# simplerr/rust-renderer

Measured on AMD Instinct MI355X. Metric: Mrays/s (path rays: primary + bounce + sun-shadow + light-shadow) at 1920x1080, 20 spp = 20 frames x 1 spp; camera and sun at rest, the one-off builds of the camera grid and the sun grid outside the timed region (value_with_grid_builds charges them to these frames, value_tree_walk uses neither grid), higher is better.
Workload: dtype f32

## Files before the change

### rust-renderer_amd/csrc/context_state.h

```cpp
#pragma once
#include <hip/hip_runtime.h>

#include <string>
#include <utility>
#include <vector>

#include "bvh.h"
#include "context_internal.h"
#include "device_types.h"
#include "grid_cache.h"
#include "utopian_hip.h"

using namespace uh;

struct HostMesh {
   std::vector<UhVertex> vertices;
   std::vector<uint32_t> indices;
   UhGpuMaterial material;
   float o2w[12];
   float w2o[9];
   bool iso = false, iso_reference = true;
   uint32_t iso_res = 0;
   float iso_lo = 0.0f, iso_hi = 0.0f;
   bool dev = false, host_valid = true;
// ... 297 lines not shown
   bool furnace = false;
   uint64_t frames = 0;
   float build_ms = 0.0f, last_frame_ms = 0.0f;
   float ms_by_kind[5] = {0, 0, 0, 0, 0};
   uint32_t trace_closest_launches = 0, trace_light_launches = 0;
   bool frame_timed = false;
   std::vector<EventPair> pending, free_events;
   uint32_t bvh_nodes = 0, bvh_tris = 0;

   bool sun_grid_enabled = true;
   uint64_t geom_version = 1;
   CachedGrid<3> sun;
   SunGridExtras sun_x;
   bool primary_implicit = true;
   bool slim_state = true;

   bool cam_grid_enabled = true;
   CachedGrid<32> cam;

   struct __attribute__((visibility("hidden"))) Tiles {
      uint32_t rank = 0, world = 1, tile = 64;
      DevBuf<uint32_t> owned_pixels;
      uint32_t n_owned = 0;
      DevBuf<float4> send, recv;
      hipEvent_t ev_compose = nullptr;
      void destroy() {
         owned_pixels.release(), send.release(), recv.release();
         if (ev_compose) (void)hipEventDestroy(ev_compose);
      }
   } tiles;
// ... 299 lines not shown
```

### rust-renderer_amd/csrc/device_types.h

```cpp
#pragma once
#include <hip/hip_runtime.h>

#include <cstdint>
#include <vector>

#include "bvh.h"
#include "frame_plan.h"
#include "path_layout.h"
#include "post_levels.h"
#include "sun_grid.h"
#include "utopian_hip.h"

namespace uh {

constexpr uint32_t kMaxBounces = 64;
constexpr uint32_t kQueueKinds = 5;
enum { Q_RAY = 0, Q_LIGHT = 1, Q_SUN_TREE = 2, Q_MISS = 3, Q_CAM_TREE = 4 };
constexpr uint32_t kLaunchSlots = kMaxBounces * 4 + 8;

constexpr uint32_t kShards = 32;
constexpr uint32_t kShardBits = 5;
static_assert((1u << kShardBits) == kShards, "kShards is a power of two");
static_assert(kLayoutShards == kShards && kLayoutShardBits == kShardBits, "path_layout.h states the same shards");
__host__ __device__ inline uint32_t shard_of_run(uint32_t run) { return (run * 0x9E3779B1u) >> (32 - kShardBits); }
// ... 331 lines not shown
struct LaunchCfg {
   hipStream_t stream;
   uint32_t num_cus;
   uint32_t closest_blocks_per_cu, shadow_blocks_per_cu;
   bool count_visits;
   uint32_t fused_blocks_per_cu = 4;
};

void launch_generate(const LaunchCfg&, const FrameParams&, const PathState&, Control*, uint32_t sample);
void launch_trace_closest(const LaunchCfg&, const SceneDev&, const PathState&, Control*, DeviceStats*, uint32_t bounce, uint32_t cursor_slot,
                          int ray_kind);
void launch_trace_camera_grid(const LaunchCfg&, const FrameParams&, const SceneDev&, const PathState&, Control*, DeviceStats*, uint32_t cursor_slot_grid, uint32_t cursor_slot_tree,
                              const SunGridDev&, bool leftovers_possible = true);
void launch_shade_miss(const LaunchCfg&, const FrameParams&, const PathState&, Control*, DeviceStats*, uint32_t bounce);
void launch_shade_hit(const LaunchCfg&, const FrameParams&, const SceneDev&, const PathState&, const Images&, Control*, DeviceStats*, uint32_t bounce);
void launch_flush_survivors(const LaunchCfg&, const FrameParams&, const PathState&, Control*);
void launch_path_fused(const LaunchCfg&, const FrameParams&, const SceneDev&, const PathState&, Control*, DeviceStats*, const SunGridDev& g, bool use_grid, bool sun_of_bounce0);
void launch_trace_shadow(const LaunchCfg&, const FrameParams&, const SceneDev&, const PathState&, Control*, DeviceStats*, uint32_t bounce,
                         uint32_t cursor_slot, bool light, bool sun_leftovers = false);
void launch_trace_sun_grid(const LaunchCfg&, const FrameParams&, const SceneDev&, const PathState&, Control*, DeviceStats*, uint32_t bounce,
                           uint32_t cursor_slot, const SunGridDev&);
void launch_finish_sample(const LaunchCfg&, const FrameParams&, const PathState&, const Images&, uint32_t sample, bool last);
void launch_resolve(const LaunchCfg&, const Images&, uint32_t W, uint32_t H, uint32_t total_samples, uint32_t limit);
void launch_gbuffer(const LaunchCfg&, const FrameParams&, const SceneDev&, const RawRays&, const Images&, DeviceStats*, const RowSpans& spans, uint32_t counted,
                    const SunGridDev* camera_grid = nullptr);
void launch_reset_reservoirs(const LaunchCfg&, const FrameParams&, const Images&, const RowSpans& spans);
void launch_initial_ris(const LaunchCfg&, const FrameParams&, const SceneDev&, const Images&, const RowSpans& spans);
void launch_temporal_reuse(const LaunchCfg&, const FrameParams&, const SceneDev&, const Images&, const RowSpans& spans);
void launch_spatial_reuse(const LaunchCfg&, const FrameParams&, const SceneDev&, const Images&, const RowSpans& spans);
void launch_trace_closest_raw(const LaunchCfg&, const SceneDev&, const float4* ray_o, const float4* ray_d, float4* hit, uint32_t n);
// ... 171 lines not shown
```

### rust-renderer_amd/csrc/frame_loop.hip

```cpp
#include <hip/hip_runtime.h>

#include <algorithm>
#include <cmath>
#include <cstring>
#include <string>

#include "context_internal.h"
#include "context_state.h"
#include "device_types.h"
#include "frame_plan.h"
#include "tile_partition.h"
#include "utopian_hip.h"

using namespace uh;

FrameParams make_params(uh_ctx* c, const UhViewUniformData& v) {
   FrameParams fp;
   std::memset(&fp, 0, sizeof(fp));
   std::memcpy(fp.inv_view, v.inverse_view, sizeof(fp.inv_view));
   std::memcpy(fp.inv_proj, v.inverse_projection, sizeof(fp.inv_proj));
   std::memcpy(fp.prev_pv, v.prev_frame_projection_view, sizeof(fp.prev_pv));
   float d = (v.sun_dir[0] * v.sun_dir[0] + v.sun_dir[1] * v.sun_dir[1]) + v.sun_dir[2] * v.sun_dir[2];
   float inv = 1.0f / std::sqrt(d);
   for (int a = 0; a < 3; a++) fp.sun_dir[a] = v.sun_dir[a] * inv;
// ... 46 lines not shown
      if (c->last_acc == s.ev_acc) c->last_acc = nullptr;
      for (hipEvent_t& r : c->spatial_reader)
         if (r == s.ev_acc) r = nullptr;
      if (c->t_start == s.frame_start) c->t_start = nullptr;
      if (c->t_stop == s.frame_stop) c->t_stop = nullptr;
      s.destroy();
   }
   HIP_TRY(c, s.create(need));
   return UH_OK;
}

static int enqueue_path_trace(uh_ctx* c, Slot& s, const FrameParams& frame) {
   FrameParams fp = frame;
   LaunchCfg lc = cfg(c);
   lc.stream = s.stream;
   const SampleOptions opt{c->fused_bounces, c->fused_always, c->sun_x.verdicts, c->slim_state, c->overlap_miss, c->overlap_shadow, lc.closest_blocks_per_cu, lc.shadow_blocks_per_cu};
   const SampleFacts facts{fp.batch_frames, fp.num_bounces, fp.samples_per_frame, fp.n_owned, s.ps.shard_cap, fp.sun_shadow_enabled == 1, fp.lights_enabled == 1,
                           c->sun.this_frame, c->cam.this_frame};
   Control* ctl = s.control.p;
   DeviceStats* st = c->dstats.p;
   for (uint32_t smp = 0; smp < fp.samples_per_frame; smp++) {
      uint32_t slot = 0;
      const bool gpu_idle = !c->last_acc || hipEventQuery(c->last_acc) == hipSuccess;
      const SamplePlan plan = plan_sample(opt, facts, gpu_idle);
      lc.closest_blocks_per_cu = plan.closest_blocks_per_cu;
      lc.shadow_blocks_per_cu = plan.shadow_blocks_per_cu;
      fp.sun_verdicts = plan.sun_verdicts ? 1u : 0u;
      fp.slim_state = plan.slim_state ? 1u : 0u;
      HIP_TRY(c, hipMemsetAsync(ctl, 0, sizeof(Control), s.stream));
      launch_generate(lc, fp, s.ps, ctl, smp);
      for (uint32_t b = 0; b < plan.wave_bounces; b++) {
         begin_timed(c, (b == 0 && plan.grid_primary) ? 3 : 0, s.stream);
         if (b == 0 && plan.grid_primary) {
            launch_trace_camera_grid(lc, fp, c->scene, s.ps, ctl, st, slot, slot + 1, c->cam.dev, c->cam.max_list_interior > std::max(c->cam.dev.walk_whole, c->cam.dev.max_walk));
            slot += 2;
         } else
            launch_trace_closest(lc, c->scene, s.ps, ctl, st, b, slot++, b == 0 ? UH_RAY_PRIMARY : UH_RAY_BOUNCE);
         end_timed(c, s.stream);
         if (plan.side_used && b > 0) HIP_TRY(c, hipStreamWaitEvent(s.stream, s.ev_shadowed, 0));
         begin_timed(c, 2, s.stream);
         launch_shade_hit(lc, fp, c->scene, s.ps, c->im, ctl, st, b);
         if (!c->overlap_miss) launch_shade_miss(lc, fp, s.ps, ctl, st, b);
         end_timed(c, s.stream);
         LaunchCfg lsh = lc;
         hipStream_t sh_stream = s.stream;
         if (plan.side_used) {
            HIP_TRY(c, hipEventRecord(s.ev_shaded, s.stream));
            HIP_TRY(c, hipStreamWaitEvent(s.side, s.ev_shaded, 0));
         }
         if (c->overlap_miss) {
            LaunchCfg ls = lc;
            ls.stream = s.side;
            begin_timed(c, 2, s.side);
            launch_shade_miss(ls, fp, s.ps, ctl, st, b);
            end_timed(c, s.side);
         }
// ... 281 lines not shown
```

### rust-renderer_amd/csrc/frame_plan.h

```cpp
#pragma once
#include <cstdint>

#include "utopian_hip.h"

namespace uh {

constexpr uint32_t kMaxBatchFrames = 32;
constexpr uint32_t kRestirBatch = 16;
constexpr uint32_t kFusedMaxPaths = 4u << 20;
constexpr uint32_t kSingleFrameBlocksPerCu = 4;

struct SampleOptions {
   bool fused_bounces, fused_always, sun_verdicts, slim_state, overlap_miss, overlap_shadow;
   uint32_t closest_blocks_per_cu, shadow_blocks_per_cu;
};
struct SampleFacts {
   uint32_t batch_frames, num_bounces, samples_per_frame, n_owned, shard_cap;
   bool sun_shadow_enabled, lights_enabled;
   bool sun_grid, camera_grid;
};
struct SamplePlan {
   bool fused;
   bool fused_sun0;
   bool sun_verdicts;
   bool slim_state;
   uint32_t closest_blocks_per_cu, shadow_blocks_per_cu;
   bool grid_primary;
   bool side_shadow;
   bool side_used;
   bool join_side;
   uint32_t wave_bounces;
   bool flush;
};

inline SamplePlan plan_sample(const SampleOptions& o, const SampleFacts& f, bool gpu_idle) {
   SamplePlan p;
   const bool lone = f.batch_frames == 1;
   p.closest_blocks_per_cu = lone && o.closest_blocks_per_cu > kSingleFrameBlocksPerCu ? kSingleFrameBlocksPerCu : o.closest_blocks_per_cu;
   p.shadow_blocks_per_cu = lone && o.shadow_blocks_per_cu > kSingleFrameBlocksPerCu ? kSingleFrameBlocksPerCu : o.shadow_blocks_per_cu;
   p.fused = o.fused_bounces && f.batch_frames == 1 && f.num_bounces >= 2 && f.num_bounces <= 64 && f.shard_cap < (1u << 23) &&
             ((gpu_idle && f.n_owned <= kFusedMaxPaths) || o.fused_always);
   p.fused_sun0 = p.fused && f.sun_shadow_enabled && !f.lights_enabled;
   p.sun_verdicts = o.sun_verdicts && f.sun_grid && f.sun_shadow_enabled && !f.lights_enabled && !p.fused;
   p.slim_state = o.slim_state && p.sun_verdicts && f.samples_per_frame == 1;
   p.grid_primary = f.camera_grid;
   p.side_shadow = o.overlap_shadow && (f.sun_shadow_enabled || f.lights_enabled);
   p.side_used = p.side_shadow || o.overlap_miss;
   p.join_side = (o.overlap_miss || o.overlap_shadow) && f.num_bounces > 0;
   p.wave_bounces = p.fused ? 1u : f.num_bounces;
   p.flush = f.num_bounces > 0 && !p.fused && !p.slim_state;
   return p;
}

inline uint32_t plan_batch_size(uint32_t option, uint64_t owned, uint32_t pass_mask) {
   uint32_t batch = option;
   if (!batch) {
      uint64_t b = (32u << 20) / (owned ? owned : 1), cap = (33u << 20) / (owned ? owned : 1);
      if (b > cap) b = cap;
      batch = (uint32_t)(b < 1 ? 1 : b);
   }
   if (batch > kMaxBatchFrames) batch = kMaxBatchFrames;
   if ((pass_mask & UH_PASS_RESTIR) && batch > kRestirBatch) batch = kRestirBatch;
   if (!(pass_mask & UH_PASS_REFERENCE_PT)) batch = 1;
   return batch;
}
// ... 8 lines not shown
```

### rust-renderer_amd/csrc/kernels.hip

```cpp
#include <hip/hip_runtime.h>

#include "device_math.h"
#include "device_types.h"
#include "grid_walk.h"
#include "kernel_common.h"
#include "path_shading.h"
#include "traversal.h"

namespace uh {

template <bool COUNT>
__global__ __launch_bounds__(kBlock, 6) void k_trace_closest(SceneDev sc, bool sharded, const float4* __restrict__ ray_o,
                                                               const float4* __restrict__ ray_d, float4* __restrict__ hit_out, uint32_t shard_cap, Control* ctl,
                                                               DeviceStats* stats, uint32_t bounce, uint32_t cursor_slot, int ray_kind, uint32_t raw_count,
                                                               const uint32_t* __restrict__ listed) {
   const bool range_in_w = !sharded;
   __shared__ uint32_t s_stack[kWavesPerBlock][kLdsStack][64];
   __shared__ RayPool<2> s_pool[kWavesPerBlock];
   const uint32_t lane = lane_id();
   const uint32_t wave = threadIdx.x >> 6;
   uint32_t* lds_col = &s_stack[wave][0][lane];
   RayPool<2>& pool = s_pool[wave];
   RaySource src;
   uint32_t seg = 0;
// ... 318 lines not shown
            if (defer[k]) st_stream(q_tree + slot, id[k]);
         }
      });
   }
   if (sx.lb == 0 && threadIdx.x == 0) {
      atomicAdd(&stats->rays[UH_RAY_SUN_SHADOW], (unsigned long long)count);
      if (COUNT) atomicAdd(&stats->shadow_nodes_visited, (unsigned long long)count);
   }
   if (COUNT) {
      atomicAdd(&stats->shadow_tris_tested, (unsigned long long)n_tris);
      atomicAdd(&stats->sun_covered_rays, (unsigned long long)n_covered);
   }
}

template <bool COUNT>
__global__ __launch_bounds__(kBlock) void k_trace_camera_grid(SceneDev sc, FrameParams fp, PathState ps, Control* ctl, DeviceStats* stats, uint32_t cursor_slot, SunGridDev g) {
   const uint32_t lane = lane_id();
   const ShardCtx sx = shard_ctx();
   const uint32_t seg = sx.shard * ps.shard_cap;
   const uint32_t* __restrict__ queue = ps.queue[0] + seg;
   const uint32_t count = ctl->q_count[qc_index(0, Q_RAY, sx.shard)];
   uint32_t* cursor = &ctl->cursor[cursor_index(cursor_slot, sx.shard)];
   const PathRecs rec = ps.set[0];
   const float4* __restrict__ tris = sc.tris;
   uint32_t* q_tree = ps.queue[3] + seg;
   uint32_t* n_tree = &ctl->q_count[qc_index(0, Q_CAM_TREE, sx.shard)];
   uint32_t n_tris = 0;
   for (;;) {
      const uint32_t base = next_batch(cursor);
      if (base >= count) break;
// ... 12 lines not shown
         defer = end - e > (g.walk_whole > g.max_walk ? g.walk_whole : g.max_walk);
         if (defer && fp.primary_implicit) {
            float4 ro, rd;
            primary_state(fp, id, ro, rd);
            st_rec(rec_quad(rec, seg + i, REC_ORIGIN), ro);
            st_rec(rec_quad(rec, seg + i, REC_DIR), rd);
         }
         if (!defer) {
            float4 ro, rd;
            if (fp.primary_implicit)
               primary_state(fp, id, ro, rd);
            else {
               ro = ld_rec(rec_quad(rec, seg + i, REC_ORIGIN));
               rd = ld_rec(rec_quad(rec, seg + i, REC_DIR));
            }
            const V3 o = v3(ro.x, ro.y, ro.z), d = v3(rd.x, rd.y, rd.z);
            Hit best;
            best.t = 10000.0f;
            best.u = best.v = 0.0f;
            best.idx = kEmptyRef;
            best.key = 0xffffffffu;
            uint2 en = make_uint2(0u, 0u);
            if (e < end) en = reinterpret_cast<const uint2*>(g.entries)[e];
            while (e < end) {
               if (sorted && -__uint_as_float(en.y) > best.t) break;
               const uint32_t pk = en.x;
               uint2 nxt = make_uint2(0u, 0u);
               if (e + 1 < end) nxt = reinterpret_cast<const uint2*>(g.entries)[e + 1];
               const float4 a = tris[kTriStride16 * (size_t)pk + 0], b = tris[kTriStride16 * (size_t)pk + 1], c = tris[kTriStride16 * (size_t)pk + 2];
               if (COUNT) n_tris++;
               tri_compute<false>(a, b, c, pk, o, d, 0.001f, INFINITY, best);
               en = nxt;
               e++;
            }
            st_rec(ps.hit + seg + i, make_float4(best.t, best.u, best.v, __uint_as_float(best.idx)));
         }
      }
      if (__ballot(defer) != 0ull) {
         const uint32_t slot = wave_append(n_tree, defer);
         if (defer) st_stream(q_tree + slot, i);
      }
   }
   if (sx.lb == 0 && threadIdx.x == 0) atomicAdd(&stats->rays[UH_RAY_PRIMARY], (unsigned long long)count);
   if (COUNT) atomicAdd(&stats->cam_tris_tested, (unsigned long long)n_tris);
}

__global__ __launch_bounds__(kBlock) void k_gbuffer_camera_grid(SceneDev sc, RawRays ps, RowSpans spans, uint32_t W, SunGridDev g) {
   const uint32_t n = spans.total();
   const float4* __restrict__ tris = sc.tris;
// ... 82 lines not shown
   const ShardCtx sx = shard_ctx();
   const uint32_t seg = sx.shard * ps.shard_cap;
   const uint2* __restrict__ queue = reinterpret_cast<const uint2*>(ps.queue[4]) + seg;
   const uint32_t count = ctl->q_count[qc_index(bounce, Q_MISS, sx.shard)];
   for (uint32_t i = sx.lb * kBlock + threadIdx.x; i < count; i += sx.nb * kBlock) {
      const uint2 e = ld_stream(queue + i);
      shade_miss_path<SLIM>(fp, ps, seg + (e.x & ~kSunLitBit), e.y, bounce, (e.x & kSunLitBit) != 0u);
   }
   if (sx.lb == 0 && threadIdx.x == 0 && count) atomicAdd(&stats->misses, (unsigned long long)count);
}

template <bool SLIM>
__global__ __launch_bounds__(kBlock, kShadeHitBlocks) void k_shade_hit(FrameParams fp, SceneDev sc, PathState ps, Control* ctl, DeviceStats* stats, uint32_t bounce) {
   __shared__ float s_lut[256];
   s_lut[threadIdx.x] = sc.unorm_lut[threadIdx.x];
   constexpr uint32_t kLdsMeshes = 192, kLdsTextures = 64;
   __shared__ MeshShade s_mesh[kLdsMeshes];
   __shared__ TexInfo s_tex[kLdsTextures];
   const uint32_t n_lds_mesh = sc.num_meshes < kLdsMeshes ? sc.num_meshes : kLdsMeshes;
   const uint32_t n_lds_tex = sc.num_textures < kLdsTextures ? sc.num_textures : kLdsTextures;
   __shared__ uint32_t s_hits;
   __shared__ uint32_t s_list[kWavesPerBlock][6][128];
   __shared__ uint32_t s_miss[kWavesPerBlock][2][128];
   if (threadIdx.x == 0) s_hits = 0;
   if (threadIdx.x < n_lds_mesh) s_mesh[threadIdx.x] = sc.meshes[threadIdx.x];
   if (threadIdx.x < n_lds_tex) s_tex[threadIdx.x] = sc.textures[threadIdx.x];
   __syncthreads();
   const ShardCtx sx = shard_ctx();
   const uint32_t seg = sx.shard * ps.shard_cap;
   const uint32_t count = ctl->q_count[qc_index(bounce, Q_RAY, sx.shard)];
   const uint32_t* __restrict__ queue = ps.queue[bounce & 1] + seg;
   const PathRecs cur = ps.set[bounce & 1], nxt = ps.set[(bounce + 1) & 1];
   uint32_t* q_next = ps.queue[(bounce + 1) & 1] + seg;
   uint32_t* n_next = &ctl->q_count[qc_index(bounce + 1, Q_RAY, sx.shard)];
   uint32_t* q_light = ps.queue[2] + seg;
   uint32_t* n_light = &ctl->q_count[qc_index(bounce, Q_LIGHT, sx.shard)];
   uint2* q_miss = reinterpret_cast<uint2*>(ps.queue[4]) + seg;
   uint32_t* n_miss = &ctl->q_count[qc_index(bounce, Q_MISS, sx.shard)];
   const uint32_t stride = sx.nb * kBlock;
   const uint32_t rounds = (count + stride - 1) / stride;
   uint32_t n_hits = 0;
   auto shade = [&](uint32_t id, uint32_t pos_lit, float4 hr, bool valid) {
      const uint32_t pos = pos_lit & ~kSunLitBit;
      const bool sun_lit = (pos_lit & kSunLitBit) != 0u;
      const uint32_t pk = __float_as_uint(hr.w);
      bool scattered = false, want_light = false;
      uint32_t slot = 0;
      float4 n_o = make_float4(0, 0, 0, 0), n_d = make_float4(0, 0, 0, 0), n_t = make_float4(0, 0, 0, 0), n_r = make_float4(0, 0, 0, 0);
      if (valid) {
         float4 ro, rd, thr4;
         if (bounce == 0 && fp.primary_implicit) {
            primary_state(fp, id, ro, rd);
            thr4 = make_float4(1.0f, 1.0f, 1.0f, 0.0f);
         } else {
            ro = ld_rec(rec_quad(cur, seg + pos, REC_ORIGIN));
            rd = ld_rec(rec_quad(cur, seg + pos, REC_DIR));
            thr4 = ld_rec(rec_quad(cur, seg + pos, REC_THR));
         }
         uint2 rng = make_uint2(__float_as_uint(ro.w), __float_as_uint(rd.w));
         if constexpr (SLIM) {
            if (bounce != 0) id = rng.x;
            rng.x = 0u;
         }
         float4 rad4 = make_float4(0.0f, 0.0f, 0.0f, 0.0f);
         if (rad_stored(fp, bounce)) rad4 = ld_rad<SLIM>(cur, seg + pos, thr4);
         const V3 ray_dir = v3(rd.x, rd.y, rd.z);
         const float t = hr.x, bu = hr.y, bv = hr.z;
         const float4* sp = sc.shade + 4 * (size_t)pk;
         float4 s0 = sp[0], s1 = sp[1], s2 = sp[2], s3 = sp[3];
         const uint32_t mesh_index = __float_as_uint(s3.w);
         MeshShade ms = lds_fetch(s_mesh + (mesh_index < kLdsMeshes ? mesh_index : kLdsMeshes - 1));
         if (mesh_index >= n_lds_mesh) ms = sc.meshes[mesh_index];
         V3 normal;
         float uu, vv;
         surface_normal_uv(s0, s1, s2, s3, bu, bv, normal, uu, vv);
         asm volatile("" : "+v"(rng.x), "+v"(rng.y), "+v"(thr4.x), "+v"(thr4.y), "+v"(thr4.z), "+v"(rad4.x), "+v"(rad4.y), "+v"(rad4.z));
         if (sun_lit) rad4 = shadow_lit<false>(thr4, rad4);
         const V3 world_normal = world_normal_of(ms, normal, ray_dir);
         V3 origin = v3(ro.x, ro.y, ro.z) + t * ray_dir;
         origin = offset_ray(origin, world_normal);
         scattered = path_scatters(ms, ray_dir, world_normal);
         const unsigned long long scat_mask = __ballot(scattered);
         const int scat_leader = __ffsll((long long)scat_mask) - 1;
         uint32_t scat_base = 0;
         V3 color = sample_texture_pre(sc, s_lut, ms.diffuse_map, uu, vv, s_tex, n_lds_tex, [&] {
            typedef __attribute__((address_space(1))) uint32_t* global_u32_t;
            global_u32_t counter = (global_u32_t)n_next;
            asm volatile("" : "+v"(counter));
            if (scattered && (int)lane_id() == scat_leader) scat_base = __hip_atomic_fetch_add(counter, (uint32_t)__popcll(scat_mask), __ATOMIC_RELAXED, __HIP_MEMORY_SCOPE_AGENT);
         });
         color = color * v3(ms.base_color[0], ms.base_color[1], ms.base_color[2]);

         uint32_t seed = rng.y;
         const V3 scatter = material_scatter(ms, ray_dir, world_normal, color, seed);
         rng.y = seed;
         if (scat_leader >= 0) slot = (uint32_t)__builtin_amdgcn_readlane((int)scat_base, scat_leader) + __builtin_amdgcn_mbcnt_hi((uint32_t)(scat_mask >> 32), __builtin_amdgcn_mbcnt_lo((uint32_t)scat_mask, 0u));

         V3 thr = v3(thr4.x, thr4.y, thr4.z) * color;
         if (!scattered) {
            st_stream(ps.radf + id, make_float4(rad4.x + thr.x, rad4.y + thr.y, rad4.z + thr.z, __uint_as_float(rng.x)));
         } else {
            float f = 0.0f;
            int light_index = 0;
            if constexpr (!SLIM)
               if (fp.lights_enabled == 1) want_light = select_light(fp, sc, id, rng.x, origin, f, light_index);
            n_o = make_float4(origin.x, origin.y, origin.z, __uint_as_float(SLIM ? id : rng.x));
            n_d = make_float4(scatter.x, scatter.y, scatter.z, __uint_as_float(rng.y));
            n_t = make_float4(thr.x, thr.y, thr.z, SLIM ? rad4.x : f);
            n_r = make_float4(rad4.x, rad4.y, rad4.z, __uint_as_float((uint32_t)light_index));
         }
      }
      uint32_t lslot = 0;
      if constexpr (!SLIM) lslot = wave_append(n_light, want_light);
      if (scattered) {
         if constexpr (!SLIM) st_stream(q_next + slot, id);
         st_rec(rec_quad(nxt, seg + slot, REC_ORIGIN), n_o);
         if (bounce + 1 < fp.num_bounces) st_rec(rec_quad(nxt, seg + slot, REC_DIR), n_d);
         st_rec(rec_quad(nxt, seg + slot, REC_THR), n_t);
         if (rad_stored(fp, bounce + 1)) {
            if constexpr (SLIM) st_rad_pair(nxt, seg + slot, n_r.y, n_r.z);
            else st_rec(rec_quad(nxt, seg + slot, REC_RAD), n_r);
         }
      }
      if (want_light) st_stream(q_light + lslot, slot);
   };
   uint32_t(*list)[128] = s_list[threadIdx.x >> 6];
   uint32_t(*missed)[128] = s_miss[threadIdx.x >> 6];
   const uint32_t lane = lane_id();
   uint32_t n_list = 0, n_missed = 0;
   const bool verdicts = bounce != 0 && fp.sun_verdicts != 0;
   auto flush_misses = [&](uint32_t n) {
      uint32_t base = 0;
      if (lane == 0) base = atomicAdd(n_miss, n);
      base = __shfl(base, 0);
      if (lane < n) st_stream(q_miss + base + lane, make_uint2(missed[0][lane], missed[1][lane]));
   };
   auto entry = [&](uint32_t k) { return make_float4(__uint_as_float(list[2][k]), __uint_as_float(list[3][k]), __uint_as_float(list[4][k]), __uint_as_float(list[5][k])); };
   for (uint32_t r = 0; r < rounds; r++) {
      const uint32_t i = r * stride + sx.lb * kBlock + threadIdx.x;
      uint32_t id = 0;
// ... 59 lines not shown
            for (int k = 0; k < 6; k++) list[k][lane] = tmp[k];
         __builtin_amdgcn_wave_barrier();
         n_list = rest;
      }
   }
   if (n_list) {
      shade(lane < n_list ? list[0][lane] : 0u, lane < n_list ? list[1][lane] : 0u, lane < n_list ? entry(lane) : make_float4(0.0f, 0.0f, 0.0f, 0.0f), lane < n_list);
      n_hits += n_list;
   }
   if (n_missed) flush_misses(n_missed);
   if (lane_id() == 0 && n_hits) atomicAdd(&s_hits, n_hits);
   __syncthreads();
   if (threadIdx.x == 0 && s_hits) atomicAdd(&stats->closest_hits, (unsigned long long)s_hits);
}

__global__ __launch_bounds__(kBlock) void k_flush_survivors(FrameParams fp, PathState ps, Control* ctl) {
   const ShardCtx sx = shard_ctx();
   const uint32_t seg = sx.shard * ps.shard_cap, b = fp.num_bounces;
   const uint32_t count = ctl->q_count[qc_index(b, Q_RAY, sx.shard)];
   const uint32_t* __restrict__ queue = ps.queue[b & 1] + seg;
   const PathRecs rec = ps.set[b & 1];
   for (uint32_t i = sx.lb * kBlock + threadIdx.x; i < count; i += sx.nb * kBlock) {
      const uint32_t id = ld_stream(queue + i);
      float4 rad = make_float4(0.0f, 0.0f, 0.0f, 0.0f);
      if (rad_stored(fp, b)) rad = ld_rec(rec_quad(rec, seg + i, REC_RAD));
      const float4 ro = ld_rec(rec_quad(rec, seg + i, REC_ORIGIN));
      if (fp.sun_verdicts) {
         const uint32_t i0 = __builtin_amdgcn_readfirstlane(i - lane_id());
         if ((*sun_lit_word(ps, seg + i0) >> lane_id()) & 1ull) rad = shadow_lit<false>(ld_rec(rec_quad(rec, seg + i, REC_THR)), rad);
      }
// ... 102 lines not shown
      k_trace_camera_grid<false><<<grid, kBlock, 0, c.stream>>>(sc, fp, ps, ctl, stats, cursor_slot_grid, g);
   if (!leftovers_possible) return;
   const PathRecs& rec = ps.set[0];
   launch_closest(c, closest_grid(c), sc, true, rec_quad(rec, 0, REC_ORIGIN), rec_quad(rec, 0, REC_DIR), ps.hit, ps.shard_cap, ctl, stats, 0, cursor_slot_tree, UH_RAY_PRIMARY, 0, ps.queue[3]);
}

void launch_shade_miss(const LaunchCfg& c, const FrameParams& fp, const PathState& ps, Control* ctl, DeviceStats* stats, uint32_t bounce) {
   const dim3 full = shade_grid(c, fp.n_owned * fp.batch_frames), lean = sharded_grid(c.num_cus * 8);
   as_constant(fp.slim_state != 0, [&](auto slim) { k_shade_miss<decltype(slim)::value><<<full.x < lean.x ? full : lean, kBlock, 0, c.stream>>>(fp, ps, ctl, stats, bounce); });
}

void launch_shade_hit(const LaunchCfg& c, const FrameParams& fp, const SceneDev& sc, const PathState& ps, const Images& im, Control* ctl,
                      DeviceStats* stats, uint32_t bounce) {
   as_constant(fp.slim_state != 0, [&](auto slim) { k_shade_hit<decltype(slim)::value><<<shade_grid(c, fp.W * fp.H), kBlock, 0, c.stream>>>(fp, sc, ps, ctl, stats, bounce); });
}
static bool final_sun_rays(const FrameParams& fp, uint32_t bounce) { return fp.slim_state != 0 && bounce + 1 == fp.num_bounces; }

void launch_flush_survivors(const LaunchCfg& c, const FrameParams& fp, const PathState& ps, Control* ctl) {
   k_flush_survivors<<<shade_grid(c, fp.n_owned * fp.batch_frames), kBlock, 0, c.stream>>>(fp, ps, ctl);
}

void launch_trace_shadow(const LaunchCfg& c, const FrameParams& fp, const SceneDev& sc, const PathState& ps, Control* ctl, DeviceStats* stats,
                         uint32_t bounce, uint32_t cursor_slot, bool light, bool sun_leftovers) {
   as_constant(c.count_visits, [&](auto count) {
      auto go = [&](auto is_light, auto verdict, auto final) {
         k_trace_shadow<decltype(count)::value, decltype(is_light)::value, decltype(verdict)::value, decltype(final)::value><<<shadow_grid(c), kBlock, 0, c.stream>>>(
            sc, fp, ps, ctl, stats, bounce, cursor_slot, sun_leftovers);
      };
      if (light) go(std::true_type{}, std::false_type{}, std::false_type{});
      else if (sun_leftovers && final_sun_rays(fp, bounce)) go(std::false_type{}, std::true_type{}, std::true_type{});
// ... 59 lines not shown
```

### rust-renderer_amd/csrc/options.hip

```cpp
#include <hip/hip_runtime.h>

#include <string>

#include "context_state.h"
#include "utopian_hip.h"

using namespace uh;

extern "C" {

int uh_set_option(uh_ctx* c, const char* name, int value) {
   if (!c) return UH_ERR_INVALID_ARGUMENT;
   if (!name) return fail(c, UH_ERR_INVALID_ARGUMENT, "null option name");
   const std::string n(name);
   auto range = [&](int lo, int hi) { return value >= lo && value <= hi; };
   auto bad = [&](const char* what) { return fail(c, UH_ERR_INVALID_ARGUMENT, n + " " + what); };
   if (n == "count_visits")
      c->count_visits = value != 0;
   else if (n == "time_kernels") {
      if (c->time_kernels && !value) {
         (void)sync_all(c);
         drain_timed(c);
      }
      c->time_kernels = value != 0;
// ... 47 lines not shown
      c->cam_grid_enabled = value != 0;
   else if (n == "camera_grid_max_walk") {
      if (!range(1, 4096)) return bad("must be 1..4096");
      c->cam.limits.max_walk = (uint32_t)value;
      c->cam.cache.invalidate();
   } else if (n == "camera_grid_walk_whole") {
      if (!range(0, 65536)) return bad("must be 0..65536");
      c->cam_walk_whole = (uint32_t)value;
      c->cam.cache.invalidate();
   } else if (n == "camera_grid_max_mean_list_x10") {
      if (!range(1, 100000)) return bad("must be 1..100000");
      c->cam.limits.max_mean_list = value / 10.0;
      c->cam.cache.invalidate();
   } else if (n == "primary_implicit")
      c->primary_implicit = value != 0;
   else if (n == "full_frame_restir")
      c->full_frame_restir = value != 0;
   else if (n == "iso_reference_triangulation")
      c->iso_reference = value != 0;
   else if (n == "furnace")
      c->furnace = value != 0;
   else if (n == "rtao_order") {
      if (!range(0, 2)) return bad("must be 0..2");
      c->hy.ao.order = (uint32_t)value;
   }
   else if (n == "rtgi_order") {
      if (!range(0, 1)) return bad("must be 0 or 1");
      c->hy.gi.order = (uint32_t)value;
   }
   else if (n == "fog_order") {
// ... 40 lines not shown
```

Before: 10470.

## Fuse primary ray generation, camera-grid trace and first-hit shading into one kernel

Adds a k_primary_shade kernel that builds each primary ray implicitly, walks its camera-grid cell list and shades the hit in the same thread. This replaces the separate generate, camera-grid trace and shade_hit launches for bounce 0. The shading body moves into a shared template with a PRIMARY flag. The aim is to drop the primary-ray hit buffer round trip and two launches per sample. The fused path only runs when the plan allows it: implicit primaries, slim state, camera lists walked fully, no visit counting and no tile partition. Otherwise the old path is used.

```diff
diff --git a/rust-renderer_amd/csrc/context_state.h b/rust-renderer_amd/csrc/context_state.h
--- a/rust-renderer_amd/csrc/context_state.h
+++ b/rust-renderer_amd/csrc/context_state.h
@@ -335,6 +335,7 @@
    SunGridExtras sun_x;
    bool primary_implicit = true;
    bool slim_state = true;
+   bool fused_primary = true;
 
    bool cam_grid_enabled = true;
    CachedGrid<32> cam;
diff --git a/rust-renderer_amd/csrc/device_types.h b/rust-renderer_amd/csrc/device_types.h
--- a/rust-renderer_amd/csrc/device_types.h
+++ b/rust-renderer_amd/csrc/device_types.h
@@ -369,6 +369,7 @@
                               const SunGridDev&, bool leftovers_possible = true);
 void launch_shade_miss(const LaunchCfg&, const FrameParams&, const PathState&, Control*, DeviceStats*, uint32_t bounce);
 void launch_shade_hit(const LaunchCfg&, const FrameParams&, const SceneDev&, const PathState&, const Images&, Control*, DeviceStats*, uint32_t bounce);
+void launch_primary_shade(const LaunchCfg&, const FrameParams&, const SceneDev&, const PathState&, Control*, DeviceStats*, const SunGridDev&);
 void launch_flush_survivors(const LaunchCfg&, const FrameParams&, const PathState&, Control*);
 void launch_path_fused(const LaunchCfg&, const FrameParams&, const SceneDev&, const PathState&, Control*, DeviceStats*, const SunGridDev& g, bool use_grid, bool sun_of_bounce0);
 void launch_trace_shadow(const LaunchCfg&, const FrameParams&, const SceneDev&, const PathState&, Control*, DeviceStats*, uint32_t bounce,
diff --git a/rust-renderer_amd/csrc/frame_loop.hip b/rust-renderer_amd/csrc/frame_loop.hip
--- a/rust-renderer_amd/csrc/frame_loop.hip
+++ b/rust-renderer_amd/csrc/frame_loop.hip
@@ -84,9 +84,11 @@
    FrameParams fp = frame;
    LaunchCfg lc = cfg(c);
    lc.stream = s.stream;
-   const SampleOptions opt{c->fused_bounces, c->fused_always, c->sun_x.verdicts, c->slim_state, c->overlap_miss, c->overlap_shadow, lc.closest_blocks_per_cu, lc.shadow_blocks_per_cu};
+   const SampleOptions opt{c->fused_bounces, c->fused_always, c->sun_x.verdicts, c->slim_state, c->overlap_miss, c->overlap_shadow, lc.closest_blocks_per_cu, lc.shadow_blocks_per_cu,
+                           c->fused_primary};
+   const bool cam_leftovers = c->cam.max_list_interior > std::max(c->cam.dev.walk_whole, c->cam.dev.max_walk);
    const SampleFacts facts{fp.batch_frames, fp.num_bounces, fp.samples_per_frame, fp.n_owned, s.ps.shard_cap, fp.sun_shadow_enabled == 1, fp.lights_enabled == 1,
-                           c->sun.this_frame, c->cam.this_frame};
+                           c->sun.this_frame, c->cam.this_frame, fp.primary_implicit != 0, c->cam.this_frame && !cam_leftovers, lc.count_visits, fp.owned_pixels != nullptr};
    Control* ctl = s.control.p;
    DeviceStats* st = c->dstats.p;
    for (uint32_t smp = 0; smp < fp.samples_per_frame; smp++) {
@@ -98,18 +100,24 @@
       fp.sun_verdicts = plan.sun_verdicts ? 1u : 0u;
       fp.slim_state = plan.slim_state ? 1u : 0u;
       HIP_TRY(c, hipMemsetAsync(ctl, 0, sizeof(Control), s.stream));
-      launch_generate(lc, fp, s.ps, ctl, smp);
+      if (!plan.fused_primary) launch_generate(lc, fp, s.ps, ctl, smp);
       for (uint32_t b = 0; b < plan.wave_bounces; b++) {
-         begin_timed(c, (b == 0 && plan.grid_primary) ? 3 : 0, s.stream);
-         if (b == 0 && plan.grid_primary) {
-            launch_trace_camera_grid(lc, fp, c->scene, s.ps, ctl, st, slot, slot + 1, c->cam.dev, c->cam.max_list_interior > std::max(c->cam.dev.walk_whole, c->cam.dev.max_walk));
+         const bool primary_shade = b == 0 && plan.fused_primary;
+         if (primary_shade)
             slot += 2;
-         } else
-            launch_trace_closest(lc, c->scene, s.ps, ctl, st, b, slot++, b == 0 ? UH_RAY_PRIMARY : UH_RAY_BOUNCE);
-         end_timed(c, s.stream);
+         else {
+            begin_timed(c, (b == 0 && plan.grid_primary) ? 3 : 0, s.stream);
+            if (b == 0 && plan.grid_primary) {
+               launch_trace_camera_grid(lc, fp, c->scene, s.ps, ctl, st, slot, slot + 1, c->cam.dev, cam_leftovers);
+               slot += 2;
+            } else
+               launch_trace_closest(lc, c->scene, s.ps, ctl, st, b, slot++, b == 0 ? UH_RAY_PRIMARY : UH_RAY_BOUNCE);
+            end_timed(c, s.stream);
+         }
          if (plan.side_used && b > 0) HIP_TRY(c, hipStreamWaitEvent(s.stream, s.ev_shadowed, 0));
          begin_timed(c, 2, s.stream);
-         launch_shade_hit(lc, fp, c->scene, s.ps, c->im, ctl, st, b);
+         if (primary_shade) launch_primary_shade(lc, fp, c->scene, s.ps, ctl, st, c->cam.dev);
+         else launch_shade_hit(lc, fp, c->scene, s.ps, c->im, ctl, st, b);
          if (!c->overlap_miss) launch_shade_miss(lc, fp, s.ps, ctl, st, b);
          end_timed(c, s.stream);
          LaunchCfg lsh = lc;
diff --git a/rust-renderer_amd/csrc/frame_plan.h b/rust-renderer_amd/csrc/frame_plan.h
--- a/rust-renderer_amd/csrc/frame_plan.h
+++ b/rust-renderer_amd/csrc/frame_plan.h
@@ -13,11 +13,16 @@
 struct SampleOptions {
    bool fused_bounces, fused_always, sun_verdicts, slim_state, overlap_miss, overlap_shadow;
    uint32_t closest_blocks_per_cu, shadow_blocks_per_cu;
+   bool fused_primary = true;
 };
 struct SampleFacts {
    uint32_t batch_frames, num_bounces, samples_per_frame, n_owned, shard_cap;
    bool sun_shadow_enabled, lights_enabled;
    bool sun_grid, camera_grid;
+   bool primary_implicit = false;
+   bool camera_lists_walked = false;
+   bool count_visits = false;
+   bool tile_partition = false;
 };
 struct SamplePlan {
    bool fused;
@@ -31,6 +36,7 @@
    bool join_side;
    uint32_t wave_bounces;
    bool flush;
+   bool fused_primary;
 };
 
 inline SamplePlan plan_sample(const SampleOptions& o, const SampleFacts& f, bool gpu_idle) {
@@ -49,6 +55,7 @@
    p.join_side = (o.overlap_miss || o.overlap_shadow) && f.num_bounces > 0;
    p.wave_bounces = p.fused ? 1u : f.num_bounces;
    p.flush = f.num_bounces > 0 && !p.fused && !p.slim_state;
+   p.fused_primary = o.fused_primary && p.grid_primary && f.primary_implicit && p.slim_state && f.camera_lists_walked && !f.count_visits && !f.tile_partition;
    return p;
 }
 
diff --git a/rust-renderer_amd/csrc/hit_shading.h b/rust-renderer_amd/csrc/hit_shading.h
--- /dev/null
+++ b/rust-renderer_amd/csrc/hit_shading.h
@@ -0,0 +1,120 @@
+#pragma once
+#include <hip/hip_runtime.h>
+
+#include "device_math.h"
+#include "device_types.h"
+#include "path_shading.h"
+
+namespace uh {
+
+constexpr uint32_t kLdsMeshes = 192, kLdsTextures = 64;
+
+struct HitShadeCtx {
+   const float* lut;
+   const MeshShade* mesh;
+   const TexInfo* tex;
+   uint32_t n_mesh, n_tex;
+   uint32_t seg;
+   PathRecs cur, nxt;
+   uint32_t* q_next;
+   uint32_t* n_next;
+   uint32_t* q_light;
+   uint32_t* n_light;
+};
+
+template <bool SLIM, bool PRIMARY = false>
+__device__ __forceinline__ void shade_hit_path(const FrameParams& fp, const SceneDev& sc, const PathState& ps, const HitShadeCtx& cx, uint32_t bounce, uint32_t id,
+                                               uint32_t pos_lit, float4 hr, bool valid, float4 primary_o = make_float4(0, 0, 0, 0),
+                                               float4 primary_d = make_float4(0, 0, 0, 0)) {
+   const uint32_t seg = cx.seg;
+   const PathRecs cur = cx.cur, nxt = cx.nxt;
+   const uint32_t pos = pos_lit & ~kSunLitBit;
+   const bool sun_lit = !PRIMARY && (pos_lit & kSunLitBit) != 0u;
+   const uint32_t pk = __float_as_uint(hr.w);
+   bool scattered = false, want_light = false;
+   uint32_t slot = 0;
+   float4 n_o = make_float4(0, 0, 0, 0), n_d = make_float4(0, 0, 0, 0), n_t = make_float4(0, 0, 0, 0), n_r = make_float4(0, 0, 0, 0);
+   if (valid) {
+      float4 ro, rd, thr4;
+      if constexpr (PRIMARY) {
+         ro = primary_o;
+         rd = primary_d;
+         thr4 = make_float4(1.0f, 1.0f, 1.0f, 0.0f);
+      } else if (bounce == 0 && fp.primary_implicit) {
+         primary_state(fp, id, ro, rd);
+         thr4 = make_float4(1.0f, 1.0f, 1.0f, 0.0f);
+      } else {
+         ro = ld_rec(rec_quad(cur, seg + pos, REC_ORIGIN));
+         rd = ld_rec(rec_quad(cur, seg + pos, REC_DIR));
+         thr4 = ld_rec(rec_quad(cur, seg + pos, REC_THR));
+      }
+      uint2 rng = make_uint2(__float_as_uint(ro.w), __float_as_uint(rd.w));
+      if constexpr (SLIM) {
+         if (bounce != 0) id = rng.x;
+         rng.x = 0u;
+      }
+      float4 rad4 = make_float4(0.0f, 0.0f, 0.0f, 0.0f);
+      if constexpr (!PRIMARY)
+         if (rad_stored(fp, bounce)) rad4 = ld_rad<SLIM>(cur, seg + pos, thr4);
+      const V3 ray_dir = v3(rd.x, rd.y, rd.z);
+      const float t = hr.x, bu = hr.y, bv = hr.z;
+      const float4* sp = sc.shade + 4 * (size_t)pk;
+      float4 s0 = sp[0], s1 = sp[1], s2 = sp[2], s3 = sp[3];
+      const uint32_t mesh_index = __float_as_uint(s3.w);
+      MeshShade ms = lds_fetch(cx.mesh + (mesh_index < kLdsMeshes ? mesh_index : kLdsMeshes - 1));
+      if (mesh_index >= cx.n_mesh) ms = sc.meshes[mesh_index];
+      V3 normal;
+      float uu, vv;
+      surface_normal_uv(s0, s1, s2, s3, bu, bv, normal, uu, vv);
+      asm volatile("" : "+v"(rng.x), "+v"(rng.y), "+v"(thr4.x), "+v"(thr4.y), "+v"(thr4.z), "+v"(rad4.x), "+v"(rad4.y), "+v"(rad4.z));
+      if (sun_lit) rad4 = shadow_lit<false>(thr4, rad4);
+      const V3 world_normal = world_normal_of(ms, normal, ray_dir);
+      V3 origin = v3(ro.x, ro.y, ro.z) + t * ray_dir;
+      origin = offset_ray(origin, world_normal);
+      scattered = path_scatters(ms, ray_dir, world_normal);
+      const unsigned long long scat_mask = __ballot(scattered);
+      const int scat_leader = __ffsll((long long)scat_mask) - 1;
+      uint32_t scat_base = 0;
+      V3 color = sample_texture_pre(sc, cx.lut, ms.diffuse_map, uu, vv, cx.tex, cx.n_tex, [&] {
+         typedef __attribute__((address_space(1))) uint32_t* global_u32_t;
+         global_u32_t counter = (global_u32_t)cx.n_next;
+         asm volatile("" : "+v"(counter));
+         if (scattered && (int)lane_id() == scat_leader) scat_base = __hip_atomic_fetch_add(counter, (uint32_t)__popcll(scat_mask), __ATOMIC_RELAXED, __HIP_MEMORY_SCOPE_AGENT);
+      });
+      color = color * v3(ms.base_color[0], ms.base_color[1], ms.base_color[2]);
+
+      uint32_t seed = rng.y;
+      const V3 scatter = material_scatter(ms, ray_dir, world_normal, color, seed);
+      rng.y = seed;
+      if (scat_leader >= 0) slot = (uint32_t)__builtin_amdgcn_readlane((int)scat_base, scat_leader) + __builtin_amdgcn_mbcnt_hi((uint32_t)(scat_mask >> 32), __builtin_amdgcn_mbcnt_lo((uint32_t)scat_mask, 0u));
+
+      V3 thr = v3(thr4.x, thr4.y, thr4.z) * color;
+      if (!scattered) {
+         st_stream(ps.radf + id, make_float4(rad4.x + thr.x, rad4.y + thr.y, rad4.z + thr.z, __uint_as_float(rng.x)));
+      } else {
+         float f = 0.0f;
+         int light_index = 0;
+         if constexpr (!SLIM)
+            if (fp.lights_enabled == 1) want_light = select_light(fp, sc, id, rng.x, origin, f, light_index);
+         n_o = make_float4(origin.x, origin.y, origin.z, __uint_as_float(SLIM ? id : rng.x));
+         n_d = make_float4(scatter.x, scatter.y, scatter.z, __uint_as_float(rng.y));
+         n_t = make_float4(thr.x, thr.y, thr.z, SLIM ? rad4.x : f);
+         n_r = make_float4(rad4.x, rad4.y, rad4.z, __uint_as_float((uint32_t)light_index));
+      }
+   }
+   uint32_t lslot = 0;
+   if constexpr (!SLIM) lslot = wave_append(cx.n_light, want_light);
+   if (scattered) {
+      if constexpr (!SLIM) st_stream(cx.q_next + slot, id);
+      st_rec(rec_quad(nxt, seg + slot, REC_ORIGIN), n_o);
+      if (bounce + 1 < fp.num_bounces) st_rec(rec_quad(nxt, seg + slot, REC_DIR), n_d);
+      st_rec(rec_quad(nxt, seg + slot, REC_THR), n_t);
+      if (rad_stored(fp, bounce + 1)) {
+         if constexpr (SLIM) st_rad_pair(nxt, seg + slot, n_r.y, n_r.z);
+         else st_rec(rec_quad(nxt, seg + slot, REC_RAD), n_r);
+      }
+   }
+   if (want_light) st_stream(cx.q_light + lslot, slot);
+}
+
+}
diff --git a/rust-renderer_amd/csrc/kernels.hip b/rust-renderer_amd/csrc/kernels.hip
--- a/rust-renderer_amd/csrc/kernels.hip
+++ b/rust-renderer_amd/csrc/kernels.hip
@@ -3,6 +3,7 @@
 #include "device_math.h"
 #include "device_types.h"
 #include "grid_walk.h"
+#include "hit_shading.h"
 #include "kernel_common.h"
 #include "path_shading.h"
 #include "traversal.h"
@@ -356,6 +357,29 @@
 }
 
 template <bool COUNT>
+__device__ __forceinline__ Hit camera_list_walk(const SunGridDev& g, const float4* __restrict__ tris, uint32_t e, uint32_t end, bool sorted, V3 o, V3 d, uint32_t& n_tris) {
+   Hit best;
+   best.t = 10000.0f;
+   best.u = best.v = 0.0f;
+   best.idx = kEmptyRef;
+   best.key = 0xffffffffu;
+   uint2 en = make_uint2(0u, 0u);
+   if (e < end) en = reinterpret_cast<const uint2*>(g.entries)[e];
+   while (e < end) {
+      if (sorted && -__uint_as_float(en.y) > best.t) break;
+      const uint32_t pk = en.x;
+      uint2 nxt = make_uint2(0u, 0u);
+      if (e + 1 < end) nxt = reinterpret_cast<const uint2*>(g.entries)[e + 1];
+      const float4 a = tris[kTriStride16 * (size_t)pk + 0], b = tris[kTriStride16 * (size_t)pk + 1], c = tris[kTriStride16 * (size_t)pk + 2];
+      if (COUNT) n_tris++;
+      tri_compute<false>(a, b, c, pk, o, d, 0.001f, INFINITY, best);
+      en = nxt;
+      e++;
+   }
+   return best;
+}
+
+template <bool COUNT>
 __global__ __launch_bounds__(kBlock) void k_trace_camera_grid(SceneDev sc, FrameParams fp, PathState ps, Control* ctl, DeviceStats* stats, uint32_t cursor_slot, SunGridDev g) {
    const uint32_t lane = lane_id();
    const ShardCtx sx = shard_ctx();
@@ -398,25 +422,7 @@
                ro = ld_rec(rec_quad(rec, seg + i, REC_ORIGIN));
                rd = ld_rec(rec_quad(rec, seg + i, REC_DIR));
             }
-            const V3 o = v3(ro.x, ro.y, ro.z), d = v3(rd.x, rd.y, rd.z);
-            Hit best;
-            best.t = 10000.0f;
-            best.u = best.v = 0.0f;
-            best.idx = kEmptyRef;
-            best.key = 0xffffffffu;
-            uint2 en = make_uint2(0u, 0u);
-            if (e < end) en = reinterpret_cast<const uint2*>(g.entries)[e];
-            while (e < end) {
-               if (sorted && -__uint_as_float(en.y) > best.t) break;
-               const uint32_t pk = en.x;
-               uint2 nxt = make_uint2(0u, 0u);
-               if (e + 1 < end) nxt = reinterpret_cast<const uint2*>(g.entries)[e + 1];
-               const float4 a = tris[kTriStride16 * (size_t)pk + 0], b = tris[kTriStride16 * (size_t)pk + 1], c = tris[kTriStride16 * (size_t)pk + 2];
-               if (COUNT) n_tris++;
-               tri_compute<false>(a, b, c, pk, o, d, 0.001f, INFINITY, best);
-               en = nxt;
-               e++;
-            }
+            const Hit best = camera_list_walk<COUNT>(g, tris, e, end, sorted, v3(ro.x, ro.y, ro.z), v3(rd.x, rd.y, rd.z), n_tris);
             st_rec(ps.hit + seg + i, make_float4(best.t, best.u, best.v, __uint_as_float(best.idx)));
          }
       }
@@ -529,7 +535,6 @@
 __global__ __launch_bounds__(kBlock, kShadeHitBlocks) void k_shade_hit(FrameParams fp, SceneDev sc, PathState ps, Control* ctl, DeviceStats* stats, uint32_t bounce) {
    __shared__ float s_lut[256];
    s_lut[threadIdx.x] = sc.unorm_lut[threadIdx.x];
-   constexpr uint32_t kLdsMeshes = 192, kLdsTextures = 64;
    __shared__ MeshShade s_mesh[kLdsMeshes];
    __shared__ TexInfo s_tex[kLdsTextures];
    const uint32_t n_lds_mesh = sc.num_meshes < kLdsMeshes ? sc.num_meshes : kLdsMeshes;
@@ -555,90 +560,8 @@
    const uint32_t stride = sx.nb * kBlock;
    const uint32_t rounds = (count + stride - 1) / stride;
    uint32_t n_hits = 0;
-   auto shade = [&](uint32_t id, uint32_t pos_lit, float4 hr, bool valid) {
-      const uint32_t pos = pos_lit & ~kSunLitBit;
-      const bool sun_lit = (pos_lit & kSunLitBit) != 0u;
-      const uint32_t pk = __float_as_uint(hr.w);
-      bool scattered = false, want_light = false;
-      uint32_t slot = 0;
-      float4 n_o = make_float4(0, 0, 0, 0), n_d = make_float4(0, 0, 0, 0), n_t = make_float4(0, 0, 0, 0), n_r = make_float4(0, 0, 0, 0);
-      if (valid) {
-         float4 ro, rd, thr4;
-         if (bounce == 0 && fp.primary_implicit) {
-            primary_state(fp, id, ro, rd);
-            thr4 = make_float4(1.0f, 1.0f, 1.0f, 0.0f);
-         } else {
-            ro = ld_rec(rec_quad(cur, seg + pos, REC_ORIGIN));
-            rd = ld_rec(rec_quad(cur, seg + pos, REC_DIR));
-            thr4 = ld_rec(rec_quad(cur, seg + pos, REC_THR));
-         }
-         uint2 rng = make_uint2(__float_as_uint(ro.w), __float_as_uint(rd.w));
-         if constexpr (SLIM) {
-            if (bounce != 0) id = rng.x;
-            rng.x = 0u;
-         }
-         float4 rad4 = make_float4(0.0f, 0.0f, 0.0f, 0.0f);
-         if (rad_stored(fp, bounce)) rad4 = ld_rad<SLIM>(cur, seg + pos, thr4);
-         const V3 ray_dir = v3(rd.x, rd.y, rd.z);
-         const float t = hr.x, bu = hr.y, bv = hr.z;
-         const float4* sp = sc.shade + 4 * (size_t)pk;
-         float4 s0 = sp[0], s1 = sp[1], s2 = sp[2], s3 = sp[3];
-         const uint32_t mesh_index = __float_as_uint(s3.w);
-         MeshShade ms = lds_fetch(s_mesh + (mesh_index < kLdsMeshes ? mesh_index : kLdsMeshes - 1));
-         if (mesh_index >= n_lds_mesh) ms = sc.meshes[mesh_index];
-         V3 normal;
-         float uu, vv;
-         surface_normal_uv(s0, s1, s2, s3, bu, bv, normal, uu, vv);
-         asm volatile("" : "+v"(rng.x), "+v"(rng.y), "+v"(thr4.x), "+v"(thr4.y), "+v"(thr4.z), "+v"(rad4.x), "+v"(rad4.y), "+v"(rad4.z));
-         if (sun_lit) rad4 = shadow_lit<false>(thr4, rad4);
-         const V3 world_normal = world_normal_of(ms, normal, ray_dir);
-         V3 origin = v3(ro.x, ro.y, ro.z) + t * ray_dir;
-         origin = offset_ray(origin, world_normal);
-         scattered = path_scatters(ms, ray_dir, world_normal);
-         const unsigned long long scat_mask = __ballot(scattered);
-         const int scat_leader = __ffsll((long long)scat_mask) - 1;
-         uint32_t scat_base = 0;
-         V3 color = sample_texture_pre(sc, s_lut, ms.diffuse_map, uu, vv, s_tex, n_lds_tex, [&] {
-            typedef __attribute__((address_space(1))) uint32_t* global_u32_t;
-            global_u32_t counter = (global_u32_t)n_next;
-            asm volatile("" : "+v"(counter));
-            if (scattered && (int)lane_id() == scat_leader) scat_base = __hip_atomic_fetch_add(counter, (uint32_t)__popcll(scat_mask), __ATOMIC_RELAXED, __HIP_MEMORY_SCOPE_AGENT);
-         });
-         color = color * v3(ms.base_color[0], ms.base_color[1], ms.base_color[2]);
-
-         uint32_t seed = rng.y;
-         const V3 scatter = material_scatter(ms, ray_dir, world_normal, color, seed);
-         rng.y = seed;
-         if (scat_leader >= 0) slot = (uint32_t)__builtin_amdgcn_readlane((int)scat_base, scat_leader) + __builtin_amdgcn_mbcnt_hi((uint32_t)(scat_mask >> 32), __builtin_amdgcn_mbcnt_lo((uint32_t)scat_mask, 0u));
-
-         V3 thr = v3(thr4.x, thr4.y, thr4.z) * color;
-         if (!scattered) {
-            st_stream(ps.radf + id, make_float4(rad4.x + thr.x, rad4.y + thr.y, rad4.z + thr.z, __uint_as_float(rng.x)));
-         } else {
-            float f = 0.0f;
-            int light_index = 0;
-            if constexpr (!SLIM)
-               if (fp.lights_enabled == 1) want_light = select_light(fp, sc, id, rng.x, origin, f, light_index);
-            n_o = make_float4(origin.x, origin.y, origin.z, __uint_as_float(SLIM ? id : rng.x));
-            n_d = make_float4(scatter.x, scatter.y, scatter.z, __uint_as_float(rng.y));
-            n_t = make_float4(thr.x, thr.y, thr.z, SLIM ? rad4.x : f);
-            n_r = make_float4(rad4.x, rad4.y, rad4.z, __uint_as_float((uint32_t)light_index));
-         }
-      }
-      uint32_t lslot = 0;
-      if constexpr (!SLIM) lslot = wave_append(n_light, want_light);
-      if (scattered) {
-         if constexpr (!SLIM) st_stream(q_next + slot, id);
-         st_rec(rec_quad(nxt, seg + slot, REC_ORIGIN), n_o);
-         if (bounce + 1 < fp.num_bounces) st_rec(rec_quad(nxt, seg + slot, REC_DIR), n_d);
-         st_rec(rec_quad(nxt, seg + slot, REC_THR), n_t);
-         if (rad_stored(fp, bounce + 1)) {
-            if constexpr (SLIM) st_rad_pair(nxt, seg + slot, n_r.y, n_r.z);
-            else st_rec(rec_quad(nxt, seg + slot, REC_RAD), n_r);
-         }
-      }
-      if (want_light) st_stream(q_light + lslot, slot);
-   };
+   const HitShadeCtx hx{s_lut, s_mesh, s_tex, n_lds_mesh, n_lds_tex, seg, cur, nxt, q_next, n_next, q_light, n_light};
+   auto shade = [&](uint32_t id, uint32_t pos_lit, float4 hr, bool valid) { shade_hit_path<SLIM>(fp, sc, ps, hx, bounce, id, pos_lit, hr, valid); };
    uint32_t(*list)[128] = s_list[threadIdx.x >> 6];
    uint32_t(*missed)[128] = s_miss[threadIdx.x >> 6];
    const uint32_t lane = lane_id();
@@ -728,6 +651,61 @@
    if (threadIdx.x == 0 && s_hits) atomicAdd(&stats->closest_hits, (unsigned long long)s_hits);
 }
 
+template <bool SLIM>
+__global__ __launch_bounds__(kBlock, kShadeHitBlocks) void k_primary_shade(FrameParams fp, SceneDev sc, PathState ps, Control* ctl, DeviceStats* stats, SunGridDev g) {
+   static_assert(SLIM, "the plan asks for this kernel under the slim state alone");
+   __shared__ float s_lut[256];
+   s_lut[threadIdx.x] = sc.unorm_lut[threadIdx.x];
+   __shared__ MeshShade s_mesh[kLdsMeshes];
+   __shared__ TexInfo s_tex[kLdsTextures];
+   const uint32_t n_lds_mesh = sc.num_meshes < kLdsMeshes ? sc.num_meshes : kLdsMeshes;
+   const uint32_t n_lds_tex = sc.num_textures < kLdsTextures ? sc.num_textures : kLdsTextures;
+   __shared__ uint32_t s_hits;
+   if (threadIdx.x == 0) s_hits = 0;
+   if (threadIdx.x < n_lds_mesh) s_mesh[threadIdx.x] = sc.meshes[threadIdx.x];
+   if (threadIdx.x < n_lds_tex) s_tex[threadIdx.x] = sc.textures[threadIdx.x];
+   __syncthreads();
+   const uint32_t n = fp.n_owned * fp.batch_frames;
+   const uint32_t lane = lane_id();
+   const uint32_t runs = (n + 63) / 64;
+   const float4* __restrict__ tris = sc.tris;
+   uint32_t n_hits = 0, n_tris = 0;
+   for (uint32_t run = blockIdx.x * kWavesPerBlock + (threadIdx.x >> 6); run < runs; run += gridDim.x * kWavesPerBlock) {
+      const uint32_t shard = __builtin_amdgcn_readfirstlane(shard_of_run(run));
+      const uint32_t seg = shard * ps.shard_cap;
+      const uint32_t id = run * 64u + lane;
+      const bool own = id < n;
+      float4 ro = make_float4(0, 0, 0, 0), rd = make_float4(0, 0, 0, 0);
+      float4 hr = make_float4(0.0f, 0.0f, 0.0f, __uint_as_float(kEmptyRef));
+      if (own) {
+         primary_state(fp, id, ro, rd);
+         const uint32_t k = id % fp.n_owned;
+         const uint32_t pix = fp.owned_pixels ? fp.owned_pixels[k] : k;
+         const uint32_t px = pix % fp.W, py = pix / fp.W;
+         const uint32_t cell = (py + 1) * g.nx + (px + 1);
+         const uint32_t e = g.cell_start[cell], end = g.cell_start[cell + 1];
+         const Hit best = camera_list_walk<false>(g, tris, e, end, end - e <= g.max_walk, v3(ro.x, ro.y, ro.z), v3(rd.x, rd.y, rd.z), n_tris);
+         hr = make_float4(best.t, best.u, best.v, __uint_as_float(best.idx));
+      }
+      const bool is_hit = __float_as_uint(hr.w) != kEmptyRef;
+      const bool is_miss = own && !is_hit;
+      if (__ballot(is_miss) != 0ull) {
+         const uint32_t slot = wave_append(&ctl->q_count[qc_index(0, Q_MISS, shard)], is_miss);
+         if (is_miss) st_stream(reinterpret_cast<uint2*>(ps.queue[4]) + seg + slot, make_uint2(0u, id));
+      }
+      const unsigned long long mask = __ballot(is_hit);
+      if (mask == 0ull) continue;
+      const HitShadeCtx hx{s_lut, s_mesh, s_tex, n_lds_mesh, n_lds_tex, seg, ps.set[0], ps.set[1], ps.queue[1] + seg, &ctl->q_count[qc_index(1, Q_RAY, shard)],
+                           ps.queue[2] + seg, &ctl->q_count[qc_index(0, Q_LIGHT, shard)]};
+      shade_hit_path<SLIM, true>(fp, sc, ps, hx, 0u, id, 0u, hr, is_hit, ro, rd);
+      n_hits += (uint32_t)__popcll(mask);
+   }
+   if (blockIdx.x == 0 && threadIdx.x == 0) atomicAdd(&stats->rays[UH_RAY_PRIMARY], (unsigned long long)n);
+   if (lane == 0 && n_hits) atomicAdd(&s_hits, n_hits);
+   __syncthreads();
+   if (threadIdx.x == 0 && s_hits) atomicAdd(&stats->closest_hits, (unsigned long long)s_hits);
+}
+
 __global__ __launch_bounds__(kBlock) void k_flush_survivors(FrameParams fp, PathState ps, Control* ctl) {
    const ShardCtx sx = shard_ctx();
    const uint32_t seg = sx.shard * ps.shard_cap, b = fp.num_bounces;
@@ -860,6 +838,9 @@
                       DeviceStats* stats, uint32_t bounce) {
    as_constant(fp.slim_state != 0, [&](auto slim) { k_shade_hit<decltype(slim)::value><<<shade_grid(c, fp.W * fp.H), kBlock, 0, c.stream>>>(fp, sc, ps, ctl, stats, bounce); });
 }
+void launch_primary_shade(const LaunchCfg& c, const FrameParams& fp, const SceneDev& sc, const PathState& ps, Control* ctl, DeviceStats* stats, const SunGridDev& g) {
+   k_primary_shade<true><<<stream_grid(c, fp.n_owned * fp.batch_frames), kBlock, 0, c.stream>>>(fp, sc, ps, ctl, stats, g);
+}
 static bool final_sun_rays(const FrameParams& fp, uint32_t bounce) { return fp.slim_state != 0 && bounce + 1 == fp.num_bounces; }
 
 void launch_flush_survivors(const LaunchCfg& c, const FrameParams& fp, const PathState& ps, Control* ctl) {
diff --git a/rust-renderer_amd/csrc/options.hip b/rust-renderer_amd/csrc/options.hip
--- a/rust-renderer_amd/csrc/options.hip
+++ b/rust-renderer_amd/csrc/options.hip
@@ -85,6 +85,8 @@
       c->cam.cache.invalidate();
    } else if (n == "primary_implicit")
       c->primary_implicit = value != 0;
+   else if (n == "fused_primary")
+      c->fused_primary = value != 0;
    else if (n == "full_frame_restir")
       c->full_frame_restir = value != 0;
    else if (n == "iso_reference_triangulation")
```

After: 10810, median of 6. 3.2% higher.
